# SimonRennotte/Data-Efficient-Reinforcement-Learning-with-Probabilistic-Model-Predictive-Control

Hardware: AMD Instinct MI355X
Metric: MPC trajectory rollouts/sec (higher is better)
Workload: dtype f64

## Files before the change

### data-efficient-reinforcement-learning-with-probabilistic-model-predictive-control_amd/_lib.py

```python
import ctypes as C
import os

_HERE = os.path.dirname(os.path.abspath(__file__))
LIB_PATH = os.environ.get("GPMPC_LIB") or os.path.join(_HERE, "libgpmpc_hip.so")

GPMPC_OK = 0
GPMPC_ERR_ARG = -1
GPMPC_ERR_NOT_PD = -2
GPMPC_ERR_HIP = -3
GPMPC_ERR_LIMIT = -4


class GpmpcError(RuntimeError):
    def __init__(self, code, msg):
        super().__init__(f"gpmpc error {code}: {msg}")
        self.code = code


class NotPositiveDefiniteError(GpmpcError):
    """Cholesky failure of K + noise*I -- the reference lets torch.linalg.cholesky's error
    propagate uncaught (rl_gp_mpc/control_objects/models/gp_model.py:427)."""


_P = C.c_void_p
# ... 11 lines not shown
    "gpmpc_get_factors": (C.c_int, [_P, C.POINTER(_P), C.POINTER(_P)]),
    "gpmpc_read_factors": (C.c_int, [_P, _P, _P, _P]),
    "gpmpc_predict": (C.c_int, [_P, _P, _I, _I, _I, _P, _P, _P, _P]),
    "gpmpc_predict_backward": (C.c_int, [_P, _P, _I, _I, _I, _P, _P, _P, _P]),
    "gpmpc_predict_cov": (C.c_int, [_P, _P, _I, _P, _I, _I, _I, _P, _P, _P]),
    "gpmpc_moments": (C.c_int, [_P, _P, _P, _I, _I, _I, _P, _P, _P, _P]),
    "gpmpc_moments_linear": (C.c_int, [_P, _P, _P, _I, _I, _I, _P, _P, _P, _P]),
    "gpmpc_moments_backward": (C.c_int, [_P, _P, _P, _I, _I, _I, _P, _P, _P, _P, _P, _P]),
    "gpmpc_moments_linear_backward": (C.c_int, [_P, _P, _P, _I, _I, _I, _P, _P, _P, _P, _P, _P]),
    "gpmpc_forget": (C.c_int, [_P, C.POINTER(_I), _I, _P]),
    "gpmpc_last_prepare_mode": (C.c_int, [_P]),
    "gpmpc_last_rollout_path": (C.c_int, [_P]),
    "gpmpc_last_grad_path": (C.c_int, [_P]),
    "gpmpc_last_cluster": (C.c_int, [_P]),
    "gpmpc_build_id": (C.c_char_p, []),
    "gpmpc_mll": (C.c_int, [_P, _P, _P, _P, _P, _P, _I, _I, _I, C.POINTER(_D), _P]),
    "gpmpc_set_option": (C.c_int, [_P, C.c_char_p, C.c_longlong]),
    "gpmpc_set_cost": (C.c_int, [_P, _P, _P, _P, _D, _I, _P, _P, _I, _I]),
    "gpmpc_rollout": (C.c_int, [_P, _P, _P, _P, _I, _I, _I, _I, _D, _P, _P, _P, _P, _P, _P]),
    "gpmpc_rollout_linear": (C.c_int, [_P, _P, _P, _P, _I, _I, _I, _I, _D, _P, _P, _P, _P, _P, _P]),
    "gpmpc_rollout_linear_feedback": (C.c_int, [_P, _P, _P, _I, _P, _P, _I, _I, _I, _I, _D, _P, _P, _P, _P, _P, _P]),
    "gpmpc_lqr_gains": (C.c_int, [_P, _P, _P, _I, _I, _I, _I, _D, _D, _P, _P, _P, _P]),
    "gpmpc_rollout_grad": (C.c_int, [_P, _P, _P, _P, _I, _I, _I, _I, _D, _P, _P, _P, _P, _P, _P, _P]),
    "gpmpc_rollout_backward": (C.c_int, [_P, _P, _P, _P, _I, _I, _I, _I, _D, _P, _P, _P, _P, _P, _P, _P, _P, _P]),
    "gpmpc_rollout_linear_backward": (C.c_int, [_P, _P, _P, _P, _I, _I, _I, _I, _D, _P, _P, _P, _P, _P, _P, _P, _P, _P]),
    "gpmpc_rollout_linear_feedback_backward": (C.c_int, [_P, _P, _P, _I, _P, _P, _I, _I, _I, _I, _D, _P, _P, _P, _P, _P, _P, _P, _P,
                                                         _P, _P]),
    "gpmpc_objective_grad_host": (C.c_int, [_P, _P, _P, _P, _I, _I, _I, _D, C.POINTER(C.POINTER(_D)), _P]),
    "gpmpc_rollout_timed": (C.c_int, [_P, _P, _P, _P, _I, _I, _I, _I, _D, _P, _I, C.POINTER(C.c_float), _P]),
    "gpmpc_cem_search": (C.c_int, [_P, _P, _P, _I, _I, _I, _I, _D, _I, _I, C.c_ulonglong, _P, _I, _P, _P, _P, _P, _P]),
    "gpmpc_cem_local": (C.c_int, [_P, _P, _P, _I, _I, _I, _I, _I, _I, _D, _I, _I, C.c_ulonglong, _P, _I, _P, _P, _P, _P, _P, _P]),
    "gpmpc_cem_merge": (C.c_int, [_P, _P, _I, _I, _I, _I, _P, _P]),
    "gpmpc_argmin_async": (C.c_int, [_P, _P, _I, C.c_longlong, _P, _I, _P, _P]),
    "gpmpc_argmin": (C.c_int, [_P, _P, _I, C.c_longlong, C.POINTER(_D), C.POINTER(C.c_longlong), _P]),
}


ABI_VERSION = 20


def load(path=LIB_PATH):
    if not os.path.exists(path):
        raise ImportError(
            f"{path} not found: the HIP extension is required (no CPU fallback). "
            "Build it with `python __graft_entry__.py` or `make -C <package>/csrc`.")
    lib = C.CDLL(path)
    for name, (res, args) in SIGNATURES.items():
        fn = getattr(lib, name)
        fn.restype = res
        fn.argtypes = args
    if lib.gpmpc_abi_version() != ABI_VERSION:
        raise ImportError(f"{path}: ABI version {lib.gpmpc_abi_version()} != expected {ABI_VERSION}; rebuild the HIP library")
    return lib


_lib = None


def lib():
    global _lib
    if _lib is None:
        _lib = load()
    return _lib
```

### data-efficient-reinforcement-learning-with-probabilistic-model-predictive-control_amd/csrc/abi.hip

```cpp
#include <cmath>
#include <cstring>
#include <new>
#include <dlfcn.h>

#include "gpmpc_internal.h"
#include "lqr_gains_plan.h"

namespace {
struct Roctx {
    int (*push)(const char*) = nullptr;
    int (*pop)() = nullptr;
    Roctx() {
        for (const char* lib : {"librocprofiler-sdk-roctx.so", "libroctx64.so"}) {
            void* hnd = dlopen(lib, RTLD_LAZY | RTLD_LOCAL);
            if (!hnd) continue;
            push = reinterpret_cast<int (*)(const char*)>(dlsym(hnd, "roctxRangePushA"));
            pop = reinterpret_cast<int (*)()>(dlsym(hnd, "roctxRangePop"));
            if (push && pop) return;
            push = nullptr; pop = nullptr;
        }
    }
};
struct Range {
    static const Roctx& api() { static Roctx r; return r; }
    explicit Range(const char* name) { if (api().push) api().push(name); }
    ~Range() { if (api().pop) api().pop(); }
    Range(const Range&) = delete;
    Range& operator=(const Range&) = delete;
};
}

using namespace gpmpc_hip;

struct gpmpc {
    Handle h;
};

#define H_(x) (&(x)->h)

static int bad(gpmpc_t* g, const char* msg) {
    if (g) g->h.err = msg;
    return GPMPC_ERR_ARG;
}

static void free_buf(Buf& b) {
    if (b.p) (void)hipFree(b.p);
    b.p = nullptr;
    b.cap = 0;
}

extern "C" {

int gpmpc_abi_version(void) { return 20; }

int gpmpc_create(gpmpc_t** out, int device_id) {
    if (!out) return GPMPC_ERR_ARG;
    *out = nullptr;
    int ndev = 0;
    if (hipGetDeviceCount(&ndev) != hipSuccess || device_id < 0 || device_id >= ndev) return GPMPC_ERR_HIP;
    if (hipSetDevice(device_id) != hipSuccess) return GPMPC_ERR_HIP;
    gpmpc_t* g = new (std::nothrow) gpmpc();
    if (!g) return GPMPC_ERR_HIP;
    g->h.device = device_id;
    hipDeviceProp_t prop;
    if (hipGetDeviceProperties(&prop, device_id) == hipSuccess) {
        g->h.num_cu = prop.multiProcessorCount;
        if (prop.maxSharedMemoryPerMultiProcessor >= 64 * 1024)
            g->h.lds_limit = (int)prop.maxSharedMemoryPerMultiProcessor;
        if (g->h.lds_limit > 160 * 1024) g->h.lds_limit = 160 * 1024;
    }
    *out = g;
    return GPMPC_OK;
}

int gpmpc_destroy(gpmpc_t* g) {
    if (!g) return GPMPC_ERR_ARG;
    Handle* h = H_(g);
    (void)hipSetDevice(h->device);
    Buf* all[] = {&h->Xt, &h->beta, &h->iK, &h->Tm, &h->ils2, &h->var, &h->logvar, &h->gram,
                  &h->linv, &h->zvec, &h->cost, &h->best, &h->xrange, &h->mono_w, &h->traj, &h->Xc, &h->Yc,
                  &h->hyp, &h->kv, &h->vv, &h->sc, &h->gradws, &h->mllws, &h->cemws, &h->tilews, &h->sepw, &h->tgradws, &h->xch, &h->hio, &h->predws, &h->predbws, &h->covws, &h->momws, &h->mombws, &h->linws, &h->linbws, &h->lqrws, &h->Xf, &h->Yf, &h->fgws, &h->spws};
    for (Buf* b : all) free_buf(*b);
    if (h->hio_host) (void)hipHostFree(h->hio_host);
    if (h->hio_flag) (void)hipHostFree(h->hio_flag);
    if (h->xch_uc) (void)hipFree(h->xch_uc);
    if (h->info) (void)hipFree(h->info);
// ... 632 lines not shown
    }
    GPMPC_HIP_CHECK(h, hipEventRecord(e1, s));
    GPMPC_HIP_CHECK(h, hipEventSynchronize(e1));
    float t = 0.f;
    GPMPC_HIP_CHECK(h, hipEventElapsedTime(&t, e0, e1));
    (void)hipEventDestroy(e0);
    (void)hipEventDestroy(e1);
    *ms = t / (float)reps;
    return rc;
}

int gpmpc_argmin(gpmpc_t* g, const double* J, int B, long long first, double* best_J, long long* best_idx, void* stream) {
    Range roctx_range("gpmpc_argmin");
    if (!g || !J || B < 1 || first < 0) return bad(g, "bad argument");
    Handle* h = H_(g);
    GPMPC_HIP_CHECK(h, hipSetDevice(h->device));
    hipStream_t s = (hipStream_t)stream;
    int rc = launch_argmin(h, J, B, first, s);
    if (rc) return rc;
    double out[2];
    GPMPC_HIP_CHECK(h, hipMemcpyAsync(out, h->best.p, sizeof out, hipMemcpyDeviceToHost, s));
    GPMPC_HIP_CHECK(h, hipStreamSynchronize(s));
    if (best_J) *best_J = out[0];
    if (best_idx) memcpy(best_idx, &out[1], sizeof(long long));
    return GPMPC_OK;
}

int gpmpc_argmin_async(gpmpc_t* g, const double* J, int B, long long first, const double* actions, int HA, double* out_dev,
                       void* stream) {
    Range roctx_range("gpmpc_argmin_async");
    if (!g || !J || !out_dev || B < 1 || first < 0 || HA < 0) return bad(g, "bad argument");
    Handle* h = H_(g);
    GPMPC_HIP_CHECK(h, hipSetDevice(h->device));
    return launch_argmin_to(h, J, B, first, actions, HA, out_dev, (hipStream_t)stream);
}

}
```

### data-efficient-reinforcement-learning-with-probabilistic-model-predictive-control_amd/csrc/gpmpc_internal.h

```cpp
#pragma once
#include <hip/hip_runtime.h>
#include <cstddef>
#include <cstdio>
#include <string>
#include <unordered_set>

#include "../../include/gpmpc.h"

namespace gpmpc_hip {

constexpr int kMaxD = GPMPC_MAX_D;
constexpr int kMaxE = GPMPC_MAX_E;
constexpr int kWave = 64;

struct ClusterMap {
    int CS, D, P, P_off, wpp, wtri, koff;
    int CSd;
    unsigned char sepown[8];
    unsigned char meanown[4];
    unsigned char dmem[32];
    unsigned char didx[32];
    __host__ __device__ int diag_owner(int ord, int slot) const { return dmem[((ord * wtri + slot) * CSd) / (D * wtri)]; }
    __host__ __device__ int off_owner(int ord, int slot) const { return ((slot * koff) / wpp + ord * koff) % CS; }
    __host__ __device__ int sep_owner(int ord) const { return sepown[ord]; }
// ... 337 lines not shown
    bool beta_partial;
    SyrkInvForm syrk;
};

struct ForgetRows {
    int k;
    int few[8];
    const int* many;
};

int ensure_rollout_tables(Handle* h, int N, int D);
int plan_rollout(const Handle& h, int N, int D, int A, int E, int H, int Bp, const RolloutRequest& req, RolloutPlan& p);
int launch_rollout(Handle* h, RolloutArgs& a, const RolloutPlan& p, hipStream_t s);
int launch_rollout(Handle* h, RolloutArgs& a, hipStream_t s);
int launch_argmin(Handle* h, const double* J, int B, long long first, hipStream_t s);
int launch_traj_cost(Handle* h, const RolloutArgs& a, double* cm, double* cv, double* J, hipStream_t s);
int ensure_sep_table(Handle* h, int D);
bool tile_path_fits(const Handle& h, int N, int D, int E);
int tile_workspace(Handle* h, RolloutArgs& a);
int launch_tile_state_init(Handle* h, const RolloutArgs& a, hipStream_t s);
int launch_pair_tiles(Handle* h, const RolloutArgs& a, int t, hipStream_t s);
bool tile_moments_supported(const Handle& h, int D, int E, int NSP);
int launch_tile_moments(Handle* h, const RolloutArgs& a, double* mom, int* done, int NSP, int NXP, hipStream_t s);
struct RolloutSeeds {
    const double* mu; const double* Sig; const double* cm; const double* cv; const double* J;
    double* mu0_bar; double* S0_bar;
    bool cost;
};
int plan_rollout_grad(Handle* h, int N, int D, int A, int E, int H, int B, int Bp, bool seeded, GradPlan& p);
int launch_rollout_grad(Handle* h, RolloutArgs& a, double* grad_out, hipStream_t s, const RolloutSeeds* seeds = nullptr);
int launch_rollout_grad_wide(Handle* h, RolloutArgs& a, double* grad_out, hipStream_t s,
                             const RolloutSeeds* seeds = nullptr);
int launch_argmin_to(Handle* h, const double* J, int B, long long first, const double* actions, int HA, double* out_dev,
                     hipStream_t s);
void plan_prepare(const Handle& h, int N, PreparePlan& p);
int run_prepare(Handle* h, const double* X, const double* Y, const double* ls, const double* os,
                const double* noise, int N, int D, int E, hipStream_t s, bool allow_reuse = true);
int run_set_factors(Handle* h, const double* X, const double* iK, const double* beta,
                    const double* ls, const double* os, int N, int D, int E, hipStream_t s);
int ensure_model_buffers(Handle* h, int N, int D, int E, bool need_factor_ws);
int run_mll(Handle* h, const double* X, const double* Y, const double* ls, const double* os, const double* noise,
            int N, int D, int E, double* out_host, hipStream_t s);
int grow(Handle* h, Buf& b, size_t need);
int run_forget(Handle* h, const int* idx_host, int k, hipStream_t s);
int run_prepare_sparse(Handle* h, const double* X, const double* Y, int N, const double* Z, int M, const double* ls, const double* os,
                       const double* noise, double jitter_rel, int D, int E, hipStream_t s);
int launch_sparse_jitter(Handle* h, const double* os, double jitter_rel, int D, double* jit, hipStream_t s);
int launch_sparse_panel(Handle* h, const double* X, int N, int M, int D, int E, int n0, int cn, int Cs, double* kuf, hipStream_t s);
int launch_sparse_accumulate(Handle* h, const double* v, const double* Y, int M, int D, int n0, int cn, int Cs, double* G,
                             double* wpart, hipStream_t s);
int launch_sparse_bmat(Handle* h, const double* G, const double* wpart, const double* noise, int M, int D, double* Bm, double* w,
                       hipStream_t s);
int launch_sparse_beta(Handle* h, const double* Yu, const double* Yb, const double* w, const double* noise, int M, int D, double* t1,
                       double* t2, double* beta, hipStream_t s);
int launch_sparse_atb_sym(Handle* h, const double* A, const double* B, int M, int D, double* C, bool ident_minus, hipStream_t s);
int launch_forget_step(Handle* h, int n, int j, int D, int ldw, hipStream_t s);
int launch_forget_pack(Handle* h, const ForgetRows& rm, int n1, int D, int E, double* Xn, double* Yn, bool tables, hipStream_t s);
int run_predict(Handle* h, const double* Xq, int M, const double* noises_host, double* mean_out, double* var_out, hipStream_t s);
int run_predict_backward(Handle* h, const double* Xq, int M, const double* mean_bar, const double* var_bar, double* Xq_bar,
                         hipStream_t s);
int run_predict_cov(Handle* h, const double* Xa, int Ma, const double* Xb, int Mb, const double* noises_host, double* out,
                    hipStream_t s);
int run_moments(Handle* h, const double* mu, const double* Sig, int P, double* M_out, double* S_out, double* V_out,
                hipStream_t s);
int run_moments_linear(Handle* h, const double* mu, const double* Sig, int P, double* M_out, double* S_out, double* V_out,
                       hipStream_t s);
int run_rollout_linear(Handle* h, const RolloutArgs& a, hipStream_t s, const double* gains = nullptr, bool per_candidate = false);
// ... 23 lines not shown
```

### data-efficient-reinforcement-learning-with-probabilistic-model-predictive-control_amd/csrc/grad.hip

```cpp
#include "grad_stream_kernel.h"
#include "grad_sep_kernel.h"
#include "moment_schedule.h"
#include <cstring>

namespace gpmpc_hip {

namespace {

constexpr int kMomThreads = 512;

template <int DP, int NXP>
int launch_moments(Handle* h, const GradArgs& g, size_t lds_bytes, hipStream_t s) {
    auto go = [&](auto kern, int nt) -> int {
        int rc = allow_full_lds(h, reinterpret_cast<const void*>(kern));
        if (rc) return rc;
        hipLaunchKernelGGL(kern, dim3(g.H, g.B, g.gz), dim3(nt), lds_bytes, s, g);
        GPMPC_HIP_CHECK(h, hipGetLastError());
        return GPMPC_OK;
    };
    if constexpr (DP <= 3) {
        if (g.share_cu) return go(pair_moments_kernel<DP, NXP, 512, 1>, 512);
        return go(pair_moments_kernel<DP, NXP, 1024, 1>, 1024);
    } else {
        return go(pair_moments_kernel<DP, NXP, kMomThreads, 1>, kMomThreads);
    }
}

struct CostSlice {
    const double* cost; double kappa; int clip, use_constraints; double* cm; double* cv; double* J;
};
template <int DP, int NXP, int NT>
__global__ __launch_bounds__(NT) void few_candidate_moments_kernel(const GradArgs p, const CostSlice cs) {
    extern __shared__ __attribute__((aligned(16))) double smem[];
    if ((int)blockIdx.z < p.gz) { pair_moments_body<DP, NXP, NT, 1>(p, smem); return; }
    if ((int)blockIdx.z == p.gz) {
        if ((int)threadIdx.x >= 64 * DP) return;
        mean_moments_body<DP, NXP>(p, smem);
        return;
    }
    if (blockIdx.x != 0 || threadIdx.x >= 64) return;
    traj_cost_body(blockIdx.y, threadIdx.x, p.mu, p.Sig, p.actions, cs.cost, p.D, p.A, p.H, cs.kappa, cs.clip, cs.use_constraints,
                   cs.cm, cs.cv, cs.J);
}

template <int DP, int NXP>
int launch_few_candidate_moments(Handle* h, const GradArgs& g, const CostSlice& cs, size_t lds_bytes, hipStream_t s) {
    constexpr int NT = DP <= 3 ? 1024 : kMomThreads;
    auto kern = few_candidate_moments_kernel<DP, NXP, NT>;
    int rc = allow_full_lds(h, reinterpret_cast<const void*>(kern));
    if (rc) return rc;
    hipLaunchKernelGGL(kern, dim3(g.H, g.B, g.gz + (cs.cost ? 2 : 1)), dim3(NT), lds_bytes, s, g, cs);
    GPMPC_HIP_CHECK(h, hipGetLastError());
    return GPMPC_OK;
}

template <int DP>
int launch_few_candidate_moments_dp(Handle* h, const GradArgs& g, const CostSlice& cs, size_t lds_bytes, hipStream_t s) {
    if (g.NXP == 1) return launch_few_candidate_moments<DP, 1>(h, g, cs, lds_bytes, s);
    return g.NXP == 2 ? launch_few_candidate_moments<DP, 2>(h, g, cs, lds_bytes, s) : launch_few_candidate_moments<DP, 6>(h, g, cs, lds_bytes, s);
}

template <int DP, int NT, bool SEEDED>
int launch_sweep(Handle* h, const std::conditional_t<SEEDED, SeededGradArgs, GradArgs>& g, size_t lds_bytes, hipStream_t s) {
    auto kern = (g.D == DP) ? adjoint_sweep_kernel<DP, NT, DP, SEEDED> : adjoint_sweep_kernel<DP, NT, 0, SEEDED>;
    int rc = allow_full_lds(h, reinterpret_cast<const void*>(kern));
    if (rc) return rc;
    hipLaunchKernelGGL(kern, dim3(g.B), dim3(NT), lds_bytes, s, g);
    GPMPC_HIP_CHECK(h, hipGetLastError());
    return GPMPC_OK;
}

template <int DP, int NXP>
int launch_moments_stream(Handle* h, const GradArgs& g, size_t lds_bytes, hipStream_t s) {
    auto kern = pair_moments_stream_kernel<DP, NXP>;
    int rc = allow_full_lds(h, reinterpret_cast<const void*>(kern));
// ... 306 lines not shown
```

### data-efficient-reinforcement-learning-with-probabilistic-model-predictive-control_amd/csrc/rollout.hip

```cpp
#include "rollout_stream_kernel.h"

namespace gpmpc_hip {

int launch_rollout_dp2(Handle*, RolloutArgs&, int, bool, size_t, hipStream_t);
int launch_rollout_dp3(Handle*, RolloutArgs&, int, bool, size_t, hipStream_t);
int launch_rollout_dp4(Handle*, RolloutArgs&, int, bool, size_t, hipStream_t);
int launch_rollout_dp6(Handle*, RolloutArgs&, int, bool, size_t, hipStream_t);
int launch_rollout_dp8(Handle*, RolloutArgs&, int, bool, size_t, hipStream_t);
int launch_rollout_dp16(Handle*, RolloutArgs&, int, bool, size_t, hipStream_t);

__global__ __launch_bounds__(64) void traj_cost_kernel(const double* __restrict__ mu, const double* __restrict__ Sig,
                                                       const double* __restrict__ actions, const double* __restrict__ cost,
                                                       int D, int A, int H, double kappa, int clip, int use_constraints,
                                                       double* __restrict__ cm_out, double* __restrict__ cv_out,
                                                       double* __restrict__ J_out) {
    traj_cost_body(blockIdx.x, threadIdx.x, mu, Sig, actions, cost, D, A, H, kappa, clip, use_constraints, cm_out, cv_out, J_out);
}

__global__ __launch_bounds__(1024) void argmin_kernel(const double* J, int B, long long first, double* out, int index_as_double,
                                                     const double* actions, int HA) {
    __shared__ long long s_best;
    __shared__ double s_v[16];
    __shared__ long long s_i[16];
    const int tid = threadIdx.x, lane = tid & 63, wave = tid >> 6;
    double bv = INFINITY;
    long long bi = -1;
    for (int i = tid; i < B; i += 1024) {
        const double v = J[i];
        if (v < bv) { bv = v; bi = i; }
    }
    for (int off = 32; off >= 1; off >>= 1) {
        const double ov = __shfl_xor(bv, off, 64);
        const long long oi = __shfl_xor(bi, off, 64);
        if (oi >= 0 && (bi < 0 || ov < bv || (ov == bv && oi < bi))) { bv = ov; bi = oi; }
    }
    if (lane == 0) { s_v[wave] = bv; s_i[wave] = bi; }
    __syncthreads();
    if (tid == 0) {
        for (int w = 1; w < 16; ++w) {
            const double ov = s_v[w];
            const long long oi = s_i[w];
            if (oi >= 0 && (bi < 0 || ov < bv || (ov == bv && oi < bi))) { bv = ov; bi = oi; }
        }
        if (first == 0 && B > 0 && J[0] != J[0]) { bv = J[0]; bi = 0; }
        if (bi < 0) bv = INFINITY;
        out[0] = bv;
        const long long gi = (bi < 0) ? -1 : bi + first;
        if (index_as_double) out[1] = (double)gi;
        else reinterpret_cast<long long*>(out)[1] = gi;
        s_best = bi < 0 ? 0 : bi;
    }
    if (actions) {
        __syncthreads();
        const long long w = s_best;
        for (int k = tid; k < HA; k += 1024) out[2 + k] = actions[w * HA + k];
    }
}

__global__ __launch_bounds__(256) void xch_zero_kernel(unsigned long long* p, size_t n) {
    for (size_t i = (size_t)blockIdx.x * 256 + threadIdx.x; i < n; i += (size_t)gridDim.x * 256)
        __hip_atomic_store(p + i, 0ull, __ATOMIC_RELAXED, __HIP_MEMORY_SCOPE_AGENT);
}

struct InlineActs { double v[kInlineActs]; };
__global__ __launch_bounds__(64) void inline_acts_kernel(double* dst, int n, const InlineActs a) {
    for (int i = threadIdx.x; i < n; i += 64) dst[i] = a.v[i];
}

static int zero_exchange(Handle* h, unsigned long long* p, size_t words, hipStream_t s) {
    const unsigned blocks = (unsigned)((words + 255) / 256 < 256 ? (words + 255) / 256 : 256);
    hipLaunchKernelGGL(xch_zero_kernel, dim3(blocks ? blocks : 1), dim3(256), 0, s, p, words);
    GPMPC_HIP_CHECK(h, hipGetLastError());
    return GPMPC_OK;
}

int launch_traj_cost(Handle* h, const RolloutArgs& a, double* cm, double* cv, double* J, hipStream_t s) {
    hipLaunchKernelGGL(traj_cost_kernel, dim3(a.B), dim3(64), 0, s, a.mu_out, a.Sig_out, a.actions, a.cost, a.D, a.A, a.H, a.kappa,
                       a.clip, a.use_constraints, cm, cv, J);
    GPMPC_HIP_CHECK(h, hipGetLastError());
    return GPMPC_OK;
}

int launch_argmin_to(Handle* h, const double* J, int B, long long first, const double* actions, int HA, double* out_dev,
                     hipStream_t s) {
    hipLaunchKernelGGL(argmin_kernel, dim3(1), dim3(1024), 0, s, J, B, first, out_dev, 1, actions, HA);
    GPMPC_HIP_CHECK(h, hipGetLastError());
    return GPMPC_OK;
}

int launch_argmin(Handle* h, const double* J, int B, long long first, hipStream_t s) {
    int rc = grow(h, h->best, 2);
    if (rc) return rc;
    hipLaunchKernelGGL(argmin_kernel, dim3(1), dim3(1024), 0, s, J, B, first, h->best.p, 0, (const double*)nullptr, 0);
    GPMPC_HIP_CHECK(h, hipGetLastError());
    return GPMPC_OK;
}

static int ensure_monomials(Handle* h, int D) {
    if (h->mono_D == D) return GPMPC_OK;
    h->sep_kmax = 0; h->mono_CM = 0;
    for (int k = 0; k < 16; ++k) h->mono_cum[k] = 0;
    h->mono_D = D;
    if (D > 4) return GPMPC_OK;
    static thread_local int ex[kMaxMono * 4];
    static thread_local double wt[kMaxMono];
    int count = 0, kmax = -1;
    for (int k = 0; k <= kMaxTaylor; ++k) {
        long long nk = 1;
        for (int i = 1; i < D; ++i) nk = nk * (k + i) / i;
        if (count + nk > kMaxMono) break;
        int a[4] = {0, 0, 0, 0};
        a[0] = k;
        for (;;) {
            double w = 1.0;
            for (int d = 0; d < 4; ++d) { ex[count * 4 + d] = a[d]; for (int e = 2; e <= a[d]; ++e) w /= (double)e; }
            wt[count++] = w;
            int i = D - 2;
            while (i >= 0 && a[i] == 0) --i;
            if (i < 0) break;
            a[i] -= 1;
            int tail = a[D - 1];
            a[D - 1] = 0;
            a[i + 1] = tail + 1;
            if (D == 1) break;
        }
        h->mono_cum[k] = count;
// ... 276 lines not shown
```

### data-efficient-reinforcement-learning-with-probabilistic-model-predictive-control_amd/csrc/rollout_kernel.h

```cpp
#pragma once
#include "device_common.h"

#if defined(GPMPC_PROF_ON)
#define GPMPC_TRACE(id) do { if (threadIdx.x == 0 && blockIdx.x == 0) { long long now_ = __builtin_readcyclecounter(); \
    prof_acc[id] += now_ - prof_last; prof_last = now_; } \
    if (CL && threadIdx.x == 0 && (blockIdx.x & 7) == 0) { long long w_ = wall_clock64(); prof_wall[id] += w_ - prof_wlast; prof_wlast = w_; } } while (0)
#else
#define GPMPC_TRACE(id) do {} while (0)
#endif

namespace gpmpc_hip {

typedef const __attribute__((address_space(3))) double* lds_cptr;
__device__ inline double lds_b64(const double* p) {
    lds_cptr q = (lds_cptr)p;
    asm volatile("" : "+v"(q));
    return *q;
}

typedef double lds_d2 __attribute__((ext_vector_type(2)));
template <int NL, int NV>
__device__ inline void lds_load_pairs(const double* rec, double (&v)[NV]) {
    static_assert(NV >= ((NL + 1) & ~1), "destination too short");
    const lds_d2* r2 = reinterpret_cast<const lds_d2*>(rec);
// ... 1552 lines not shown
            const double v = s_mu[i] + s_M[i];
            s_mu[i] = v;
            if (member == 0) p.mu_out[((size_t)c * (H + 1) + (t + 1)) * D + i] = v;
        }
        cur ^= 1;
        __syncthreads();
        if constexpr (CL) {
            if (*s_fail) {
                if (member == 0) {
                    for (int i = tid; i < (H - t) * D; i += NT) p.mu_out[((size_t)c * (H + 1) + (t + 1)) * D + i] = __builtin_nan("");
                    for (int i = tid; i < (H - t) * D * D; i += NT) p.Sig_out[((size_t)c * (H + 1) + (t + 1)) * D * D + i] = __builtin_nan("");
                }
                return;
            }
        }
        GPMPC_TRACE(6);
    }
#if defined(GPMPC_PROF_ON)
    if (threadIdx.x == 0 && blockIdx.x == 0) printf("PROF wave0 small algebra cycles %lld\n", prof_acc[7]);
    if (blockIdx.x == 0 && threadIdx.x == 64) printf("PROF P1 pair problems done after %lld cycles (summed over steps)\n", prof_x[0]);
    if (blockIdx.x == 0 && threadIdx.x == NT - 1) printf("PROF P1 last thread done after %lld\n", prof_x[1]);
    if (blockIdx.x == 0 && (threadIdx.x & 63) == 0) printf("PROF P3 wave %d left the queue after %lld\n", (int)(threadIdx.x >> 6), prof_x[2]);
    if (CL && threadIdx.x == 0 && (blockIdx.x & 7) == 0)
        printf("PROF member %2d xcc %d same_xcd %d\n", member, (int)__builtin_amdgcn_s_getreg(20 | (0 << 6) | ((4 - 1) << 11)), (int)same_xcd);
    if (CL && threadIdx.x == 0 && (blockIdx.x & 7) == 0)
        printf("PROF member %2d wall (10 ns ticks): P1 %lld | P2 %lld | items(wave 0) %lld | gather+wait %lld | P4 %lld | P5 %lld\n", member,
               prof_wall[2], prof_wall[3], prof_wall[8], prof_wall[4], prof_wall[5], prof_wall[6]);
    if (threadIdx.x == 0 && blockIdx.x == 0)
        printf("PROF cycles: init %lld | P1 %lld | P2 %lld | P3 %lld (wave 0's items %lld) | P4 %lld | P5 %lld\n", prof_acc[1], prof_acc[2],
               prof_acc[3], prof_acc[4] + prof_acc[8], prof_acc[8], prof_acc[5], prof_acc[6]);
#endif
}

__device__ __forceinline__ void traj_cost_body(int c, int lane, const double* __restrict__ mu, const double* __restrict__ Sig,
                                                       const double* __restrict__ actions, const double* __restrict__ cost,
                                                       int D, int A, int H, double kappa, int clip, int use_constraints,
                                                       double* __restrict__ cm_out, double* __restrict__ cv_out,
                                                       double* __restrict__ J_out) {
    const int DA = D + A;
    const double* target = cost;
    const double* W = cost + DA;
    const double* WT = W + DA * DA;
    const double* smin = WT + D * D;
    const double* smax = smin + D;
    double jsum = 0.0;
    for (int t = lane; t <= H; t += 64) {
        const bool terminal = (t == H);
        const int n = terminal ? D : DA;
        const double* Wm = terminal ? WT : W;
        const double* m = mu + ((size_t)c * (H + 1) + t) * D;
        const double* S = Sig + ((size_t)c * (H + 1) + t) * D * D;
        const double* a = actions + ((size_t)c * H + (terminal ? 0 : t)) * A;
        auto err = [&](int i) { return (i < D ? m[i] : a[i - D]) - target[i]; };
        double cm = 0.0, cv = 0.0;
        for (int i = 0; i < D; ++i)
            for (int j = 0; j < D; ++j) cm = fma(S[i * D + j], Wm[j * n + i], cm);
        for (int i = 0; i < n; ++i) {
            const double ei = err(i);
            for (int j = 0; j < n; ++j) cm = fma(ei * Wm[i * n + j], err(j), cm);
        }
        for (int i = 0; i < D; ++i)
            for (int j = 0; j < D; ++j) {
                double tij = 0.0, tji = 0.0;
                for (int k = 0; k < D; ++k) {
                    tij = fma(Wm[i * n + k], S[k * D + j], tij);
                    tji = fma(Wm[j * n + k], S[k * D + i], tji);
                }
                cv = fma(2.0 * tij, tji, cv);
                double v1 = 0.0, v2 = 0.0;
                for (int k = 0; k < n; ++k) {
                    v1 = fma(err(k), Wm[k * n + i], v1);
                    v2 = fma(Wm[j * n + k], err(k), v2);
                }
                cv = fma(4.0 * v1 * S[i * D + j], v2, cv);
            }
        if (use_constraints && !terminal) {
            for (int d = 0; d < D; ++d) {
                const double sg = S[d * D + d];
                cm += 0.5 * (1.0 + erf((smin[d] - m[d]) / (sg * 1.4142135623730951)))
                    + (1.0 - 0.5 * (1.0 + erf((smax[d] - m[d]) / (sg * 1.4142135623730951))));
            }
        }
        double ucb = -cm + kappa * sqrt(cv);
        if (clip) ucb = fmin(ucb, 0.0);
        jsum -= ucb;
        if (cm_out) cm_out[(size_t)c * (H + 1) + t] = cm;
        if (cv_out) cv_out[(size_t)c * (H + 1) + t] = cv;
    }
    jsum = wave_xor_sum(jsum);
    if (lane == 0 && J_out) J_out[c] = jsum / (double)(H + 1);
}

}
```

### data-efficient-reinforcement-learning-with-probabilistic-model-predictive-control_amd/engine.py

```python
import ctypes as C

import numpy as np
import torch

from . import _lib as L


def _host(a, shape=None):
    a = np.ascontiguousarray(np.asarray(a, dtype=np.float64))
    if shape is not None and a.shape != tuple(shape):
        raise ValueError(f"expected shape {tuple(shape)}, got {a.shape}")
    return a


def _hp(a):
    return a.ctypes.data_as(C.c_void_p)


def feedback_gains_layout(shape, B, H, A, D):
    shape = tuple(int(s) for s in shape)
    if shape == (A, D):
        return False, True
    if shape == (H, A, D):
        return False, False
# ... 600 lines not shown
                                              nz.data_ptr() if nz is not None else None, best.data_ptr(), self._stream()))
        host = best.cpu().numpy()
        return host[:n].copy(), float(host[n])

    def cem_local(self, mu0, S0, B_total, first, B_local, H, A, iteration, n_elite, state, seed=0, include_time=False,
                  time0=0.0, first_candidate=None, max_change=None, action_prev=None, noise=None, out=None):
        D = self.D
        mu0 = _host(mu0, (D,))
        S0 = _host(S0, (D, D))
        n = H * A
        if out is None:
            out = torch.empty((n_elite, n + 2), dtype=torch.float64, device=self.device)
        first_c = _host(first_candidate, (n,)) if first_candidate is not None else None
        mapper = 0 if max_change is None else 1
        mc = _host(max_change, (A,)) if mapper else None
        ap = _host(action_prev, (A,)) if mapper else None
        nz = None if noise is None else self._dev(noise)
        if nz is not None and (nz.dim() != 3 or nz.shape[1] != B_total or nz.shape[2] != n):
            raise ValueError("noise must be (iterations, B_total, H*A)")
        self._check(self.lib.gpmpc_cem_local(self._h, _hp(mu0), _hp(S0), int(B_total), int(first), int(B_local), H, A,
                                             int(bool(include_time)), float(time0), int(iteration), int(n_elite),
                                             int(seed) & (2 ** 64 - 1), _hp(first_c) if first_c is not None else None, mapper,
                                             _hp(mc) if mapper else None, _hp(ap) if mapper else None,
                                             nz.data_ptr() if nz is not None else None, state.data_ptr(), out.data_ptr(),
                                             self._stream()))
        self._keep_cem = (nz, state)
        return out

    def cem_merge(self, elites, n_elite, n, iteration, state):
        lists = elites.numel() // (n_elite * (n + 2))
        self._check(self.lib.gpmpc_cem_merge(self._h, elites.data_ptr(), lists, int(n_elite), int(n), int(iteration),
                                             state.data_ptr(), self._stream()))

    def argmin_async(self, J, first_global_index=0, actions=None, out=None):
        J = self._dev(J)
        ha = 0 if actions is None else int(actions[0].numel())
        if out is None:
            out = torch.empty(2 + ha, dtype=torch.float64, device=self.device)
        self._check(self.lib.gpmpc_argmin_async(self._h, J.data_ptr(), J.numel(), int(first_global_index),
                                                None if actions is None else actions.data_ptr(), ha,
                                                out.data_ptr(), self._stream()))
        return out

    def argmin(self, J, first_global_index=0):
        J = self._dev(J)
        bj = C.c_double()
        bi = C.c_longlong()
        self._check(self.lib.gpmpc_argmin(self._h, J.data_ptr(), J.numel(), int(first_global_index), C.byref(bj),
                                          C.byref(bi), self._stream()))
        return float(bj.value), int(bi.value)
```

### data-efficient-reinforcement-learning-with-probabilistic-model-predictive-control_amd/sharding.py

```python
import math

import numpy as np
import torch
import torch.distributed as dist

LOCAL = "local"
CEM_MAX_RECORDS = 4096
_CEM_FAILED = 2147483646.0


def _active(group):
    return group is not LOCAL and dist.is_available() and dist.is_initialized()


def broadcast_from_first(array, device, group=None):
    a = np.ascontiguousarray(array, dtype=np.float64)
    if not _active(group):
        return a.copy()
    t = torch.as_tensor(a).to(device)
    src = dist.get_global_rank(group, 0) if group is not None else 0
    dist.broadcast(t, src=src, group=group)
    return t.cpu().numpy().reshape(a.shape)


# ... 127 lines not shown

class PendingBest:

    def __init__(self, host, event, world, H, A, record=None, exchange_group=None):
        self.host, self.event, self.world, self.H, self.A = host, event, world, H, A
        self.record = record
        self.exchange_group = exchange_group
        self._result = None
        self._flat = None
        self.host_seconds = None

    def result(self):
        if self._result is not None:
            return self._result
        import time
        t0 = time.perf_counter()
        if self.event is not None:
            self.event.synchronize()
        host = self.host
        if self.exchange_group is not None:
            mine = host.clone()
            flat = torch.empty(self.world * mine.numel(), dtype=torch.float64)
            dist.all_gather_into_tensor(flat, mine, group=self.exchange_group)
            host = flat
        self._result = _winner_of(host.view(self.world, -1), self.world, self.H, self.A)
        self._flat = None
        self.host_seconds = time.perf_counter() - t0
        return self._result


def select_best_async(engine, J, actions_local, lo, num_candidates, group=None, host_buffer=None, record=None,
                      exchange="rccl"):
    n, H, A = actions_local.shape
    rec = _local_record(engine, J, actions_local, lo, out=record)
    multi = _active(group)
    if exchange == "host" and multi:
        world = dist.get_world_size(group)
        xg = host_group(group)
        if rec.device.type != "cuda":
            return PendingBest(rec.clone(), None, world, H, A, rec, exchange_group=xg)
        if host_buffer is None or host_buffer.numel() != rec.numel():
            host_buffer = torch.empty(rec.numel(), dtype=torch.float64, pin_memory=True)
        host_buffer.copy_(rec, non_blocking=True)
        ev = torch.cuda.Event()
        ev.record(torch.cuda.current_stream(rec.device))
        return PendingBest(host_buffer, ev, world, H, A, rec, exchange_group=xg)
    if exchange == "rccl_side" and multi and rec.device.type == "cuda":
        world = dist.get_world_size(group)
        side = side_stream(rec.device)
        if host_buffer is None or host_buffer.numel() != world * rec.numel():
            host_buffer = torch.empty(world * rec.numel(), dtype=torch.float64, pin_memory=True)
        flat = torch.empty(world * rec.numel(), dtype=torch.float64, device=rec.device)
        work = dist.all_gather_into_tensor(flat, rec.contiguous(), group=group, async_op=True)
        with torch.cuda.stream(side):
            work.wait()
            host_buffer.copy_(flat, non_blocking=True)
            ev = torch.cuda.Event()
            ev.record(side)
        flat.record_stream(side)
        pend = PendingBest(host_buffer, ev, world, H, A, rec)
        pend._flat = flat
        return pend
    world, flat = _gather_records(rec, group)
    if rec.device.type != "cuda":
        return PendingBest(flat.clone(), None, world, H, A, rec)
    if host_buffer is None or host_buffer.numel() != flat.numel():
        host_buffer = torch.empty(flat.numel(), dtype=torch.float64, pin_memory=True)
    host_buffer.copy_(flat, non_blocking=True)
# ... 75 lines not shown
```

### include/gpmpc.h

```cpp
#ifndef GPMPC_H
#define GPMPC_H
#ifdef __cplusplus
extern "C" {
#endif

typedef struct gpmpc gpmpc_t;

enum {
    GPMPC_OK = 0,
    GPMPC_ERR_ARG = -1,
    GPMPC_ERR_NOT_PD = -2,
    GPMPC_ERR_HIP = -3,
    GPMPC_ERR_LIMIT = -4
};
#define GPMPC_MAX_D 16
#define GPMPC_MAX_E 24

int gpmpc_abi_version(void);
const char* gpmpc_build_id(void);
int gpmpc_create(gpmpc_t** out, int device_id);
int gpmpc_destroy(gpmpc_t* h);
const char* gpmpc_last_error(const gpmpc_t* h);

int gpmpc_prepare(gpmpc_t* h, const double* X_dev, const double* Y_dev, const double* lengthscales_dev,
// ... 60 lines not shown
int gpmpc_lqr_gains(gpmpc_t* h, const double* actions_dev, const double* mu0_host, int B, int H, int A, int include_time,
                    double time0, double reg, double* gains_out_dev, double* P_out_dev, int* flags_out_dev, void* stream);

int gpmpc_rollout_grad(gpmpc_t* h, const double* actions_dev, const double* mu0_host, const double* S0_host, int B, int H, int A,
                       int include_time, double time0, double* J_out_dev, double* grad_out_dev, double* mu_out_dev,
                       double* Sig_out_dev, double* cost_mu_out_dev, double* cost_var_out_dev, void* stream);
int gpmpc_last_grad_path(gpmpc_t* h);

int gpmpc_rollout_backward(gpmpc_t* h, const double* actions_dev, const double* mu0_host, const double* S0_host, int B, int H, int A,
                           int include_time, double time0, const double* mu_bar_dev, const double* Sig_bar_dev,
                           const double* cost_mu_bar_dev, const double* cost_var_bar_dev, const double* J_bar_dev,
                           double* actions_bar_out_dev, double* mu0_bar_out_dev, double* S0_bar_out_dev, void* stream);

int gpmpc_rollout_linear_backward(gpmpc_t* h, const double* actions_dev, const double* mu0_host, const double* S0_host, int B,
                                  int H, int A, int include_time, double time0, const double* mu_bar_dev,
                                  const double* Sig_bar_dev, const double* cost_mu_bar_dev, const double* cost_var_bar_dev,
                                  const double* J_bar_dev, double* actions_bar_out_dev, double* mu0_bar_out_dev,
                                  double* S0_bar_out_dev, void* stream);

int gpmpc_rollout_linear_feedback_backward(gpmpc_t* h, const double* actions_dev, const double* gains_dev, int gains_per_candidate,
                                           const double* mu0_host, const double* S0_host, int B, int H, int A, int include_time,
                                           double time0, const double* mu_bar_dev, const double* Sig_bar_dev,
                                           const double* cost_mu_bar_dev, const double* cost_var_bar_dev, const double* J_bar_dev,
                                           double* actions_bar_out_dev, double* gains_bar_out_dev, double* mu0_bar_out_dev,
                                           double* S0_bar_out_dev, void* stream);

int gpmpc_objective_grad_host(gpmpc_t* h, const double* actions_host, const double* mu0_host, const double* S0_host,
                              int H, int A, int include_time, double time0, const double** result_host, void* stream);

int gpmpc_argmin(gpmpc_t* h, const double* J_dev, int B, long long first_global_index, double* best_J_host,
                 long long* best_idx_host, void* stream);
int gpmpc_argmin_async(gpmpc_t* h, const double* J_dev, int B, long long first_global_index, const double* actions_dev, int HA,
                       double* out_dev, void* stream);

int gpmpc_cem_search(gpmpc_t* h, const double* mu0_host, const double* S0_host, int B, int H, int A, int include_time, double time0,
                     int iterations, int n_elite, unsigned long long seed, const double* first_candidate_host, int mapper,
                     const double* max_change_host, const double* action_prev_host, const double* noise_dev, double* best_out_dev,
                     void* stream);
int gpmpc_cem_local(gpmpc_t* h, const double* mu0_host, const double* S0_host, int B_total, int first, int B_local, int H, int A,
                    int include_time, double time0, int iteration, int n_elite, unsigned long long seed,
                    const double* first_candidate_host, int mapper, const double* max_change_host, const double* action_prev_host,
                    const double* noise_dev, const double* state_dev, double* elites_out_dev, void* stream);
int gpmpc_cem_merge(gpmpc_t* h, const double* elites_dev, int lists, int n_elite, int n, int iteration, double* state_dev,
                    void* stream);

int gpmpc_rollout_timed(gpmpc_t* h, const double* actions_dev, const double* mu0_host, const double* S0_host, int B, int H, int A,
                        int include_time, double time0, double* J_out_dev, int reps, float* ms_host, void* stream);

#ifdef __cplusplus
}
#endif
#endif
```

Measured before the change: 674,000.

## Write argmin result to pinned host memory, size argmin block, specialize cost kernel

Adds an argmin export path in which the kernel writes the best cost, index and actions directly into pinned, device-mapped host memory, so the separate device-to-host copy is skipped in single-device selection. The argmin block now scales with B, and the cross-wave reduction moves from a serial loop on one thread to wave shuffles. The trajectory cost body also gets compile-time specializations for small D/A, with W and S held in registers and the loops unrolled. The costs are a new ABI version, more register pressure in the cost kernels, and host-mapped writes that need a system fence.

```diff
diff --git a/data-efficient-reinforcement-learning-with-probabilistic-model-predictive-control_amd/_lib.py b/data-efficient-reinforcement-learning-with-probabilistic-model-predictive-control_amd/_lib.py
--- a/data-efficient-reinforcement-learning-with-probabilistic-model-predictive-control_amd/_lib.py
+++ b/data-efficient-reinforcement-learning-with-probabilistic-model-predictive-control_amd/_lib.py
@@ -67,11 +67,12 @@
     "gpmpc_cem_local": (C.c_int, [_P, _P, _P, _I, _I, _I, _I, _I, _I, _D, _I, _I, C.c_ulonglong, _P, _I, _P, _P, _P, _P, _P, _P]),
     "gpmpc_cem_merge": (C.c_int, [_P, _P, _I, _I, _I, _I, _P, _P]),
     "gpmpc_argmin_async": (C.c_int, [_P, _P, _I, C.c_longlong, _P, _I, _P, _P]),
+    "gpmpc_argmin_export": (C.c_int, [_P, _P, _I, C.c_longlong, _P, _I, _P, _P, _P]),
     "gpmpc_argmin": (C.c_int, [_P, _P, _I, C.c_longlong, C.POINTER(_D), C.POINTER(C.c_longlong), _P]),
 }
 
 
-ABI_VERSION = 20
+ABI_VERSION = 21
 
 
 def load(path=LIB_PATH):
diff --git a/data-efficient-reinforcement-learning-with-probabilistic-model-predictive-control_amd/csrc/abi.hip b/data-efficient-reinforcement-learning-with-probabilistic-model-predictive-control_amd/csrc/abi.hip
--- a/data-efficient-reinforcement-learning-with-probabilistic-model-predictive-control_amd/csrc/abi.hip
+++ b/data-efficient-reinforcement-learning-with-probabilistic-model-predictive-control_amd/csrc/abi.hip
@@ -51,7 +51,7 @@
 
 extern "C" {
 
-int gpmpc_abi_version(void) { return 20; }
+int gpmpc_abi_version(void) { return 21; }
 
 int gpmpc_create(gpmpc_t** out, int device_id) {
     if (!out) return GPMPC_ERR_ARG;
@@ -750,7 +750,23 @@
     if (!g || !J || !out_dev || B < 1 || first < 0 || HA < 0) return bad(g, "bad argument");
     Handle* h = H_(g);
     GPMPC_HIP_CHECK(h, hipSetDevice(h->device));
-    return launch_argmin_to(h, J, B, first, actions, HA, out_dev, (hipStream_t)stream);
-}
-
-}
+    return launch_argmin_to(h, J, B, first, actions, HA, out_dev, nullptr, (hipStream_t)stream);
+}
+
+int gpmpc_argmin_export(gpmpc_t* g, const double* J, int B, long long first, const double* actions, int HA, double* out_dev,
+                        double* out_host, void* stream) {
+    Range roctx_range("gpmpc_argmin_export");
+    if (!g || !J || !out_dev || !out_host || B < 1 || first < 0 || HA < 0) return bad(g, "bad argument");
+    Handle* h = H_(g);
+    GPMPC_HIP_CHECK(h, hipSetDevice(h->device));
+    hipPointerAttribute_t attr;
+    void* dev_view = nullptr;
+    if (hipPointerGetAttributes(&attr, out_host) != hipSuccess || attr.type != hipMemoryTypeHost ||
+        hipHostGetDevicePointer(&dev_view, out_host, 0) != hipSuccess || !dev_view) {
+        (void)hipGetLastError();
+        return bad(g, "out_host must be pinned (page-locked, device-mapped) host memory");
+    }
+    return launch_argmin_to(h, J, B, first, actions, HA, out_dev, static_cast<double*>(dev_view), (hipStream_t)stream);
+}
+
+}
diff --git a/data-efficient-reinforcement-learning-with-probabilistic-model-predictive-control_amd/csrc/gpmpc_internal.h b/data-efficient-reinforcement-learning-with-probabilistic-model-predictive-control_amd/csrc/gpmpc_internal.h
--- a/data-efficient-reinforcement-learning-with-probabilistic-model-predictive-control_amd/csrc/gpmpc_internal.h
+++ b/data-efficient-reinforcement-learning-with-probabilistic-model-predictive-control_amd/csrc/gpmpc_internal.h
@@ -393,7 +393,7 @@
 int launch_rollout_grad_wide(Handle* h, RolloutArgs& a, double* grad_out, hipStream_t s,
                              const RolloutSeeds* seeds = nullptr);
 int launch_argmin_to(Handle* h, const double* J, int B, long long first, const double* actions, int HA, double* out_dev,
-                     hipStream_t s);
+                     double* out_host, hipStream_t s);
 void plan_prepare(const Handle& h, int N, PreparePlan& p);
 int run_prepare(Handle* h, const double* X, const double* Y, const double* ls, const double* os,
                 const double* noise, int N, int D, int E, hipStream_t s, bool allow_reuse = true);
diff --git a/data-efficient-reinforcement-learning-with-probabilistic-model-predictive-control_amd/csrc/grad.hip b/data-efficient-reinforcement-learning-with-probabilistic-model-predictive-control_amd/csrc/grad.hip
--- a/data-efficient-reinforcement-learning-with-probabilistic-model-predictive-control_amd/csrc/grad.hip
+++ b/data-efficient-reinforcement-learning-with-probabilistic-model-predictive-control_amd/csrc/grad.hip
@@ -39,8 +39,8 @@
         return;
     }
     if (blockIdx.x != 0 || threadIdx.x >= 64) return;
-    traj_cost_body(blockIdx.y, threadIdx.x, p.mu, p.Sig, p.actions, cs.cost, p.D, p.A, p.H, cs.kappa, cs.clip, cs.use_constraints,
-                   cs.cm, cs.cv, cs.J);
+    traj_cost_body<DP>(blockIdx.y, threadIdx.x, p.mu, p.Sig, p.actions, cs.cost, p.D, p.A, p.H, cs.kappa, cs.clip, cs.use_constraints,
+                       cs.cm, cs.cv, cs.J);
 }
 
 template <int DP, int NXP>
diff --git a/data-efficient-reinforcement-learning-with-probabilistic-model-predictive-control_amd/csrc/rollout.hip b/data-efficient-reinforcement-learning-with-probabilistic-model-predictive-control_amd/csrc/rollout.hip
--- a/data-efficient-reinforcement-learning-with-probabilistic-model-predictive-control_amd/csrc/rollout.hip
+++ b/data-efficient-reinforcement-learning-with-probabilistic-model-predictive-control_amd/csrc/rollout.hip
@@ -17,44 +17,58 @@
     traj_cost_body(blockIdx.x, threadIdx.x, mu, Sig, actions, cost, D, A, H, kappa, clip, use_constraints, cm_out, cv_out, J_out);
 }
 
+__device__ __forceinline__ void keep_better(double& bv, long long& bi, double ov, long long oi) {
+    if (oi >= 0 && (bi < 0 || ov < bv || (ov == bv && oi < bi))) { bv = ov; bi = oi; }
+}
+
 __global__ __launch_bounds__(1024) void argmin_kernel(const double* J, int B, long long first, double* out, int index_as_double,
-                                                     const double* actions, int HA) {
-    __shared__ long long s_best;
+                                                     const double* actions, int HA, double* out_host) {
     __shared__ double s_v[16];
     __shared__ long long s_i[16];
-    const int tid = threadIdx.x, lane = tid & 63, wave = tid >> 6;
+    const int tid = threadIdx.x, lane = tid & 63, wave = tid >> 6, nt = blockDim.x, nw = nt >> 6;
+    const double j0 = B > 0 ? J[0] : 0.0;
     double bv = INFINITY;
     long long bi = -1;
-    for (int i = tid; i < B; i += 1024) {
+    for (int i = tid; i < B; i += nt) {
         const double v = J[i];
         if (v < bv) { bv = v; bi = i; }
     }
     for (int off = 32; off >= 1; off >>= 1) {
         const double ov = __shfl_xor(bv, off, 64);
         const long long oi = __shfl_xor(bi, off, 64);
-        if (oi >= 0 && (bi < 0 || ov < bv || (ov == bv && oi < bi))) { bv = ov; bi = oi; }
-    }
-    if (lane == 0) { s_v[wave] = bv; s_i[wave] = bi; }
-    __syncthreads();
+        keep_better(bv, bi, ov, oi);
+    }
+    if (nw > 1) {
+        if (lane == 0) { s_v[wave] = bv; s_i[wave] = bi; }
+        __syncthreads();
+        bv = lane < nw ? s_v[lane] : INFINITY;
+        bi = lane < nw ? s_i[lane] : -1;
+        for (int off = 8; off >= 1; off >>= 1) {
+            const double ov = __shfl_xor(bv, off, 64);
+            const long long oi = __shfl_xor(bi, off, 64);
+            keep_better(bv, bi, ov, oi);
+        }
+        bv = __shfl(bv, 0, 64);
+        bi = __shfl(bi, 0, 64);
+    }
+    if (first == 0 && B > 0 && j0 != j0) { bv = j0; bi = 0; }
+    if (bi < 0) bv = INFINITY;
     if (tid == 0) {
-        for (int w = 1; w < 16; ++w) {
-            const double ov = s_v[w];
-            const long long oi = s_i[w];
-            if (oi >= 0 && (bi < 0 || ov < bv || (ov == bv && oi < bi))) { bv = ov; bi = oi; }
-        }
-        if (first == 0 && B > 0 && J[0] != J[0]) { bv = J[0]; bi = 0; }
-        if (bi < 0) bv = INFINITY;
+        const long long gi = (bi < 0) ? -1 : bi + first;
         out[0] = bv;
-        const long long gi = (bi < 0) ? -1 : bi + first;
         if (index_as_double) out[1] = (double)gi;
         else reinterpret_cast<long long*>(out)[1] = gi;
-        s_best = bi < 0 ? 0 : bi;
+        if (out_host) { out_host[0] = bv; out_host[1] = (double)gi; }
     }
     if (actions) {
-        __syncthreads();
-        const long long w = s_best;
-        for (int k = tid; k < HA; k += 1024) out[2 + k] = actions[w * HA + k];
-    }
+        const long long w = bi < 0 ? 0 : bi;
+        for (int k = tid; k < HA; k += nt) {
+            const double v = actions[w * HA + k];
+            out[2 + k] = v;
+            if (out_host) out_host[2 + k] = v;
+        }
+    }
+    if (out_host) __threadfence_system();
 }
 
 __global__ __launch_bounds__(256) void xch_zero_kernel(unsigned long long* p, size_t n) {
@@ -81,9 +95,14 @@
     return GPMPC_OK;
 }
 
+static inline int argmin_threads(int B) {
+    const int w = (B + 63) / 64;
+    return 64 * (w < 1 ? 1 : w > 16 ? 16 : w);
+}
+
 int launch_argmin_to(Handle* h, const double* J, int B, long long first, const double* actions, int HA, double* out_dev,
-                     hipStream_t s) {
-    hipLaunchKernelGGL(argmin_kernel, dim3(1), dim3(1024), 0, s, J, B, first, out_dev, 1, actions, HA);
+                     double* out_host, hipStream_t s) {
+    hipLaunchKernelGGL(argmin_kernel, dim3(1), dim3(argmin_threads(B)), 0, s, J, B, first, out_dev, 1, actions, HA, out_host);
     GPMPC_HIP_CHECK(h, hipGetLastError());
     return GPMPC_OK;
 }
@@ -91,7 +110,8 @@
 int launch_argmin(Handle* h, const double* J, int B, long long first, hipStream_t s) {
     int rc = grow(h, h->best, 2);
     if (rc) return rc;
-    hipLaunchKernelGGL(argmin_kernel, dim3(1), dim3(1024), 0, s, J, B, first, h->best.p, 0, (const double*)nullptr, 0);
+    hipLaunchKernelGGL(argmin_kernel, dim3(1), dim3(argmin_threads(B)), 0, s, J, B, first, h->best.p, 0, (const double*)nullptr, 0,
+                       (double*)nullptr);
     GPMPC_HIP_CHECK(h, hipGetLastError());
     return GPMPC_OK;
 }
diff --git a/data-efficient-reinforcement-learning-with-probabilistic-model-predictive-control_amd/csrc/rollout_kernel.h b/data-efficient-reinforcement-learning-with-probabilistic-model-predictive-control_amd/csrc/rollout_kernel.h
--- a/data-efficient-reinforcement-learning-with-probabilistic-model-predictive-control_amd/csrc/rollout_kernel.h
+++ b/data-efficient-reinforcement-learning-with-probabilistic-model-predictive-control_amd/csrc/rollout_kernel.h
@@ -1608,11 +1608,11 @@
 #endif
 }
 
-__device__ __forceinline__ void traj_cost_body(int c, int lane, const double* __restrict__ mu, const double* __restrict__ Sig,
-                                                       const double* __restrict__ actions, const double* __restrict__ cost,
-                                                       int D, int A, int H, double kappa, int clip, int use_constraints,
-                                                       double* __restrict__ cm_out, double* __restrict__ cv_out,
-                                                       double* __restrict__ J_out) {
+__device__ __forceinline__ void traj_cost_generic(int c, int lane, const double* __restrict__ mu, const double* __restrict__ Sig,
+                                                          const double* __restrict__ actions, const double* __restrict__ cost,
+                                                          int D, int A, int H, double kappa, int clip, int use_constraints,
+                                                          double* __restrict__ cm_out, double* __restrict__ cv_out,
+                                                          double* __restrict__ J_out) {
     const int DA = D + A;
     const double* target = cost;
     const double* W = cost + DA;
@@ -1667,4 +1667,114 @@
     if (lane == 0 && J_out) J_out[c] = jsum / (double)(H + 1);
 }
 
-}
+template <int D, int N>
+__device__ __forceinline__ void stage_cost_terms(const double* S, const double* e, const double* Wm, double& cm_out, double& cv_out) {
+    double cm = 0.0, cv = 0.0;
+#pragma unroll
+    for (int i = 0; i < D; ++i)
+#pragma unroll
+        for (int j = 0; j < D; ++j) cm = fma(S[i * D + j], Wm[j * N + i], cm);
+#pragma unroll
+    for (int i = 0; i < N; ++i) {
+        const double ei = e[i];
+#pragma unroll
+        for (int j = 0; j < N; ++j) cm = fma(ei * Wm[i * N + j], e[j], cm);
+    }
+#pragma unroll
+    for (int i = 0; i < D; ++i)
+#pragma unroll
+        for (int j = 0; j < D; ++j) {
+            double tij = 0.0, tji = 0.0;
+#pragma unroll
+            for (int k = 0; k < D; ++k) {
+                tij = fma(Wm[i * N + k], S[k * D + j], tij);
+                tji = fma(Wm[j * N + k], S[k * D + i], tji);
+            }
+            cv = fma(2.0 * tij, tji, cv);
+            double v1 = 0.0, v2 = 0.0;
+#pragma unroll
+            for (int k = 0; k < N; ++k) {
+                v1 = fma(e[k], Wm[k * N + i], v1);
+                v2 = fma(Wm[j * N + k], e[k], v2);
+            }
+            cv = fma(4.0 * v1 * S[i * D + j], v2, cv);
+        }
+    cm_out = cm;
+    cv_out = cv;
+}
+
+template <int D, int A>
+__device__ __forceinline__ void traj_cost_fixed(int c, int lane, const double* __restrict__ mu, const double* __restrict__ Sig,
+                                                        const double* __restrict__ actions, const double* __restrict__ cost,
+                                                        int H, double kappa, int clip, int use_constraints,
+                                                        double* __restrict__ cm_out, double* __restrict__ cv_out,
+                                                        double* __restrict__ J_out) {
+    constexpr int DA = D + A;
+    double target[DA], W[DA * DA], WT[D * D], smin[D], smax[D];
+#pragma unroll
+    for (int i = 0; i < DA; ++i) target[i] = cost[i];
+#pragma unroll
+    for (int i = 0; i < DA * DA; ++i) W[i] = cost[DA + i];
+#pragma unroll
+    for (int i = 0; i < D * D; ++i) WT[i] = cost[DA + DA * DA + i];
+#pragma unroll
+    for (int d = 0; d < D; ++d) {
+        smin[d] = cost[DA + DA * DA + D * D + d];
+        smax[d] = cost[DA + DA * DA + D * D + D + d];
+    }
+    double jsum = 0.0;
+    for (int t = lane; t <= H; t += 64) {
+        const bool terminal = (t == H);
+        const double* mp = mu + ((size_t)c * (H + 1) + t) * D;
+        const double* Sp = Sig + ((size_t)c * (H + 1) + t) * D * D;
+        const double* ap = actions + ((size_t)c * H + (terminal ? 0 : t)) * A;
+        double S[D * D], m[D], e[DA];
+#pragma unroll
+        for (int i = 0; i < D * D; ++i) S[i] = Sp[i];
+#pragma unroll
+        for (int i = 0; i < D; ++i) m[i] = mp[i];
+#pragma unroll
+        for (int i = 0; i < A; ++i) e[D + i] = (terminal ? 0.0 : ap[i]) - target[D + i];
+#pragma unroll
+        for (int i = 0; i < D; ++i) e[i] = m[i] - target[i];
+        double cm, cv;
+        if (terminal) stage_cost_terms<D, D>(S, e, WT, cm, cv);
+        else stage_cost_terms<D, DA>(S, e, W, cm, cv);
+        if (use_constraints && !terminal) {
+#pragma unroll
+            for (int d = 0; d < D; ++d) {
+                const double sg = S[d * D + d];
+                cm += 0.5 * (1.0 + erf((smin[d] - m[d]) / (sg * 1.4142135623730951)))
+                    + (1.0 - 0.5 * (1.0 + erf((smax[d] - m[d]) / (sg * 1.4142135623730951))));
+            }
+        }
+        double ucb = -cm + kappa * sqrt(cv);
+        if (clip) ucb = fmin(ucb, 0.0);
+        jsum -= ucb;
+        if (cm_out) cm_out[(size_t)c * (H + 1) + t] = cm;
+        if (cv_out) cv_out[(size_t)c * (H + 1) + t] = cv;
+    }
+    jsum = wave_xor_sum(jsum);
+    if (lane == 0 && J_out) J_out[c] = jsum / (double)(H + 1);
+}
+
+template <int DPAD = 0>
+__device__ __forceinline__ void traj_cost_body(int c, int lane, const double* __restrict__ mu, const double* __restrict__ Sig,
+                                                       const double* __restrict__ actions, const double* __restrict__ cost,
+                                                       int D, int A, int H, double kappa, int clip, int use_constraints,
+                                                       double* __restrict__ cm_out, double* __restrict__ cv_out,
+                                                       double* __restrict__ J_out) {
+#define GPMPC_COST_FIXED(d, a)                                                                                                    \
+    if constexpr (DPAD == 0 || (DPAD == 2 ? (d) <= 2 : (d) == DPAD)) {                                                            \
+        if (D == (d) && A == (a)) {                                                                                               \
+            traj_cost_fixed<d, a>(c, lane, mu, Sig, actions, cost, H, kappa, clip, use_constraints, cm_out, cv_out, J_out);       \
+            return;                                                                                                               \
+        }                                                                                                                         \
+    }
+    GPMPC_COST_FIXED(1, 1) GPMPC_COST_FIXED(1, 2) GPMPC_COST_FIXED(2, 1) GPMPC_COST_FIXED(2, 2)
+    GPMPC_COST_FIXED(3, 1) GPMPC_COST_FIXED(3, 2) GPMPC_COST_FIXED(4, 1) GPMPC_COST_FIXED(4, 2)
+#undef GPMPC_COST_FIXED
+    traj_cost_generic(c, lane, mu, Sig, actions, cost, D, A, H, kappa, clip, use_constraints, cm_out, cv_out, J_out);
+}
+
+}
diff --git a/data-efficient-reinforcement-learning-with-probabilistic-model-predictive-control_amd/engine.py b/data-efficient-reinforcement-learning-with-probabilistic-model-predictive-control_amd/engine.py
--- a/data-efficient-reinforcement-learning-with-probabilistic-model-predictive-control_amd/engine.py
+++ b/data-efficient-reinforcement-learning-with-probabilistic-model-predictive-control_amd/engine.py
@@ -656,14 +656,24 @@
         self._check(self.lib.gpmpc_cem_merge(self._h, elites.data_ptr(), lists, int(n_elite), int(n), int(iteration),
                                              state.data_ptr(), self._stream()))
 
-    def argmin_async(self, J, first_global_index=0, actions=None, out=None):
+    argmin_exports_host = True
+
+    def argmin_async(self, J, first_global_index=0, actions=None, out=None, host_out=None):
         J = self._dev(J)
         ha = 0 if actions is None else int(actions[0].numel())
         if out is None:
             out = torch.empty(2 + ha, dtype=torch.float64, device=self.device)
-        self._check(self.lib.gpmpc_argmin_async(self._h, J.data_ptr(), J.numel(), int(first_global_index),
-                                                None if actions is None else actions.data_ptr(), ha,
-                                                out.data_ptr(), self._stream()))
+        if host_out is None:
+            self._check(self.lib.gpmpc_argmin_async(self._h, J.data_ptr(), J.numel(), int(first_global_index),
+                                                    None if actions is None else actions.data_ptr(), ha,
+                                                    out.data_ptr(), self._stream()))
+            return out
+        if (host_out.device.type != "cpu" or host_out.dtype != torch.float64 or not host_out.is_contiguous()
+                or host_out.numel() != 2 + ha or not host_out.is_pinned()):
+            raise ValueError("host_out must be a pinned contiguous float64 host tensor of 2 + H*A elements")
+        self._check(self.lib.gpmpc_argmin_export(self._h, J.data_ptr(), J.numel(), int(first_global_index),
+                                                 None if actions is None else actions.data_ptr(), ha,
+                                                 out.data_ptr(), host_out.data_ptr(), self._stream()))
         return out
 
     def argmin(self, J, first_global_index=0):
diff --git a/data-efficient-reinforcement-learning-with-probabilistic-model-predictive-control_amd/sharding.py b/data-efficient-reinforcement-learning-with-probabilistic-model-predictive-control_amd/sharding.py
--- a/data-efficient-reinforcement-learning-with-probabilistic-model-predictive-control_amd/sharding.py
+++ b/data-efficient-reinforcement-learning-with-probabilistic-model-predictive-control_amd/sharding.py
@@ -183,8 +183,15 @@
 def select_best_async(engine, J, actions_local, lo, num_candidates, group=None, host_buffer=None, record=None,
                       exchange="rccl"):
     n, H, A = actions_local.shape
+    multi = _active(group)
+    if (not multi and n > 0 and actions_local.device.type == "cuda" and getattr(engine, "argmin_exports_host", False)):
+        if host_buffer is None or host_buffer.numel() != 2 + H * A:
+            host_buffer = torch.empty(2 + H * A, dtype=torch.float64, pin_memory=True)
+        rec = engine.argmin_async(J, first_global_index=lo, actions=actions_local, out=record, host_out=host_buffer)
+        ev = torch.cuda.Event()
+        ev.record(torch.cuda.current_stream(rec.device))
+        return PendingBest(host_buffer, ev, 1, H, A, rec)
     rec = _local_record(engine, J, actions_local, lo, out=record)
-    multi = _active(group)
     if exchange == "host" and multi:
         world = dist.get_world_size(group)
         xg = host_group(group)
diff --git a/include/gpmpc.h b/include/gpmpc.h
--- a/include/gpmpc.h
+++ b/include/gpmpc.h
@@ -116,6 +116,8 @@
                  long long* best_idx_host, void* stream);
 int gpmpc_argmin_async(gpmpc_t* h, const double* J_dev, int B, long long first_global_index, const double* actions_dev, int HA,
                        double* out_dev, void* stream);
+int gpmpc_argmin_export(gpmpc_t* h, const double* J_dev, int B, long long first_global_index, const double* actions_dev, int HA,
+                        double* out_dev, double* out_host, void* stream);
 
 int gpmpc_cem_search(gpmpc_t* h, const double* mu0_host, const double* S0_host, int B, int H, int A, int include_time, double time0,
                      int iterations, int n_elite, unsigned long long seed, const double* first_candidate_host, int mapper,
```

Measured after the change: 701,400 (median of 6 runs). 4.1% higher.
